# DreamOneX/yet-another-bpe

Measured on AMD Instinct MI355X. Metric: merges_per_sec, higher is better.
Workload: dtype u16

## Files before the change

include/yabpe.h:

```cpp
#ifndef YABPE_H
#define YABPE_H

#include <stddef.h>
#include <stdint.h>

#ifdef __cplusplus
extern "C" {
#endif

#define YABPE_ABI_VERSION 2

enum {
    YABPE_OK = 0,
    YABPE_E_INVALID = -1,
    YABPE_E_NODEVICE = -2,
    YABPE_E_HIP = -3,
    YABPE_E_CAPACITY = -4,
    YABPE_E_INTERNAL = -5,
    YABPE_E_COMM = -6,
    YABPE_E_UTF8 = -7
};

#define YABPE_LOAD_DEDUP 0x1u

// ... 45 lines not shown
    uint64_t retiles, table_rebuilds;
    double load_ms;
    double train_ms;
    double apply_ms_sampled;
    uint64_t apply_launches_sampled;
    uint64_t apply_algo_bytes_sampled;
    uint64_t apply_actual_bytes_sampled;
    uint64_t algo_bytes_total;
    double scan_ms_sampled;
    uint64_t scan_launches_sampled;
    uint64_t scan_algo_bytes_sampled;
    uint64_t scan_actual_bytes_sampled;
    uint64_t scan_skip_launches;
    uint64_t scan_skip_tiles_read;
    uint64_t cand_rebuilds;
    uint64_t cand_rescans;
    uint64_t fused_launches;
    double dense_ms_sampled;
    uint64_t dense_launches_sampled;
    uint64_t dense_algo_bytes_sampled;
    uint64_t dense_actual_bytes_sampled;
    double sparse_ms;
    uint64_t sparse_merges;
    double tail_ms;
    uint64_t tail_merges;
    uint64_t exchanges, exchange_bytes, exchange_cap_records, exchange_growths, exchange_max_records;
    uint64_t sparse_launches;
    uint64_t tail_launches;
    double exchange_ms_sampled;
    uint64_t exchanges_sampled;
    uint64_t exchange_p2p;
    uint64_t dense_launches, dense_merges;
    uint64_t scan_skip_pieces_taken;
} yabpe_stats_t;
int yabpe_stats(yabpe_ctx *ctx, yabpe_stats_t *out);
int yabpe_iter_log(yabpe_ctx *ctx, uint64_t *out_sites, uint64_t *out_live_slots, uint32_t cap, uint32_t *out_n);

int yabpe_event_log(yabpe_ctx *ctx, uint32_t *out_iter, float *out_us, float *out_scan_us, uint32_t cap, uint32_t *out_n);

typedef struct yabpe_latency_t {
    double launch_gap_us;
    double load_trip_us;
    double coherent_trip_us;
    double atomic_trip_us;
} yabpe_latency_t;
int yabpe_latency_probe(yabpe_ctx *ctx, yabpe_latency_t *out);

int yabpe_verify_table(yabpe_ctx *ctx, uint64_t *out_mismatches);
int yabpe_stream_checksum(yabpe_ctx *ctx, uint64_t *out_sum, uint64_t *out_words, uint64_t *out_tokens);

int yabpe_synth_generate(yabpe_ctx *ctx, uint64_t target_bytes, uint32_t n_types, uint64_t seed,
                         const uint8_t *alphabet, uint32_t alphabet_len, int space_prefix,
                         uint8_t **out_dev_bytes, uint64_t **out_dev_off, uint64_t *out_n_words, uint64_t *out_n_bytes);
int yabpe_synth_generate_lex(yabpe_ctx *ctx, uint64_t target_bytes, uint32_t n_types, uint64_t seed,
                             const uint8_t *lex_bytes, const uint64_t *lex_off,
                             uint8_t **out_dev_bytes, uint64_t **out_dev_off, uint64_t *out_n_pieces, uint64_t *out_n_bytes);
int yabpe_synth_free(yabpe_ctx *ctx);
int yabpe_memcpy_d2h(yabpe_ctx *ctx, void *dst_host, const void *src_dev, uint64_t n);
int yabpe_memcpy_h2d(yabpe_ctx *ctx, void *dst_dev, const void *src_host, uint64_t n);

int yabpe_pretokenize(yabpe_ctx *ctx, const uint8_t *text, uint64_t n_bytes, const uint64_t *chunk_off, uint32_t n_chunks,
                      const uint8_t *special_bytes, const uint32_t *special_off, uint32_t n_special,
                      const uint8_t **out_dev_text, uint64_t **out_dev_word_off, uint64_t *out_n_words, int64_t *out_bad_pos);
int yabpe_pretokenize_free(yabpe_ctx *ctx);

int yabpe_pool_add(yabpe_ctx *ctx, const uint8_t *bytes, const uint64_t *word_off, const uint64_t *word_freq, uint64_t n_words);
// ... 109 lines not shown
```

yet-another-bpe_amd/csrc/yabpe.hip:

```cpp
#include <hip/hip_runtime.h>
#include <dlfcn.h>
#include <rccl/rccl.h>

#include <algorithm>
#include <cstdarg>
#include <cstddef>
#include <cstdio>
#include <cstring>
#include <map>
#include <mutex>
#include <string>
#include <vector>

#include "../../include/yabpe.h"
#include "yabpe_kernels.h"
#include "yabpe_aux_kernels.h"
#include "yabpe_devmem.h"
#include "yabpe_pretok_kernels.h"
#include "yabpe_encode_kernels.h"
#include "yabpe_dropout_kernels.h"
#include "yabpe_decode_kernels.h"
#include "yabpe_layout_kernels.h"
#include "yabpe_replay_kernels.h"
#include "yabpe_pool_kernels.h"
// ... 61 lines not shown
}

struct yabpe_ctx {
    int device = 0;
    int n_cu = 256;
    int apply_occ = 4;
    hipStream_t stream = nullptr;
    std::string err;
    std::map<std::string, int64_t> opt;

    bool have_vocab = false;
    uint32_t base_tokens = 0;
    TokTable tt{};
    bool have_words = false;
    bool weighted = false;
    uint64_t n_words = 0, n_words_input = 0, tokens_initial = 0;
    uint32_t n_tiles = 0;
    uint16_t *tiles = nullptr, *tiles_alt = nullptr;
    uint32_t tiles_cap = 0, tiles_alt_cap = 0;
    uint32_t *tile_len = nullptr, *tile_len_alt = nullptr;
    uint32_t *tile_wbase = nullptr, *tile_wbase_alt = nullptr;
    uint32_t *wfreq = nullptr;
    uint32_t n_long = 0;
    uint16_t *long_tok = nullptr;
    unsigned long long *long_sig = nullptr;
    uint32_t long_sig_stride = 0;
    unsigned long long *long_off = nullptr;
    uint32_t *long_len = nullptr, *long_freq = nullptr;
    uint64_t long_tokens = 0;
    PairTable table{};
    uint64_t table_cap = 0;
    DevState *st = nullptr;
    DevState *st_host = nullptr;
    Best *partials = nullptr;
    uint32_t n_partials = 0, n_partials_cap = 0;
    uint32_t rec_cap = 0, rec_n = 0;
    uint32_t *rec_left = nullptr, *rec_right = nullptr, *rec_merged = nullptr;
    unsigned long long *rec_count = nullptr, *rec_sites = nullptr, *rec_live = nullptr;
    std::vector<uint64_t> log_sites, log_live;
    std::vector<uint32_t> ev_iter;
    std::vector<float> ev_us;
    yabpe_stats_t stats{};
    std::vector<EventPair> events;
    std::vector<void *> synth_bufs;
    std::vector<void *> pretok_bufs;
    uint8_t *pt_cls = nullptr;
    bool have_enc_model = false;
    unsigned long long *enc_keys = nullptr;
    uint32_t *enc_vals = nullptr;
    unsigned long long enc_mask = 0;
    uint32_t *enc_out_id = nullptr;
    uint8_t *enc_sp_bytes = nullptr, *enc_sp_has = nullptr;
    uint32_t *enc_sp_off = nullptr, *enc_sp_id = nullptr;
    uint32_t enc_n_special = 0, enc_sp_max_len = 0;
    uint32_t *enc_ids = nullptr;
    unsigned long long *enc_doc = nullptr;
    unsigned long long *enc_spans = nullptr;
    yabpe_encode_stats_t enc_stats{};
    unsigned long long enc_sums[4] = {0, 0, 0, 0};
    bool enc_done = false;
    hipEvent_t enc_ev[8] = {};
    bool have_dec_model = false;
    uint2 *dec_ent = nullptr;
    uint8_t *dec_pool = nullptr;
    uint32_t dec_n = 0;
    uint8_t *dec_text = nullptr;
    unsigned long long *dec_doc = nullptr;
    yabpe_decode_stats_t dec_stats{};
    hipEvent_t dec_ev[7] = {};
    uint32_t *lay_buf[3] = {};
    yabpe_layout_stats_t lay_stats{};
    hipEvent_t lay_ev[4] = {};
    yabpe_resume_stats_t resume_stats{};
    bool have_pool = false;
    PoolView wpool{};
    uint64_t wpool_arena_cap = 0, wpool_n = 0, wpool_bytes = 0;
    yabpe_pool_stats_t wpool_stats{};
    hipEvent_t wpool_ev[4] = {};
    unsigned long long *scratch64 = nullptr;
    unsigned long long *blk_stats = nullptr;
    uint32_t blk_used = 0;
    bool split_mode = false;
    uint32_t kmax_now = 1;
    uint32_t rec_n_live = 0;
    std::vector<float> ev_scan_us;
    unsigned long long *sig = nullptr;
    uint32_t sig_stride = 0;
    unsigned long long *blk_read = nullptr;
    uint64_t scan_skip_launches = 0;
    uint64_t piece_tag = 0;
    bool sig_valid = false;
    uint32_t sig_built_at = 0;
    uint64_t sig_tokens_at_build = 0;
    uint64_t sig_builds = 0;
    CandState *cand_state = nullptr;
    uint32_t cand_built_at = 0;
    unsigned long long cand_best_at_build = 0;
    uint32_t *sel_ticket = nullptr;
    unsigned long long *cand = nullptr;
    bool use_cand = false;
    uint64_t cand_rebuilds = 0, cand_rescans = 0;
    double cand_margin = 0.2;
    uint32_t cand_n_at_build = 0;
    bool pending = false;
    uint64_t fused_launches = 0;
    int rank = 0, n_ranks = 1;
    bool multi = false;
    ncclComm_t comm = nullptr;
    yabpe_allgather_fn ag_fn = nullptr;
    void *ag_user = nullptr;
    unsigned long long *xsmall = nullptr;
    uint8_t *xsend = nullptr, *xrecv = nullptr;
    uint64_t exchange_growths = 0;
    uint64_t exchange_max_records = 0;
    uint32_t xcap = 0;
    uint64_t xstride = 0;
    uint32_t xeff = 0;
    uint64_t xeff_sum = 0;
    uint32_t xseen[4] = {0, 0, 0, 0};
    uint64_t exchanges = 0;
    bool p2p = false;
    uint8_t *p2p_area = nullptr;
    std::vector<uint8_t *> p2p_peer;
    uint64_t p2p_half = 0, p2p_flags_off = 0, p2p_seq = 0, p2p_stride = 0;
    uint32_t p2p_cap = 0;
    hipEvent_t p2p_e0 = nullptr, p2p_e1 = nullptr;
    bool p2p_pending = false;
};
// ... 96 lines not shown
    t.sink_rec = nullptr;
    t.sink_hdr = nullptr;
    t.sink_cap = 0;
}

int table_alloc(yabpe_ctx *c, PairTable &t, uint64_t cap, unsigned long long *entries_ctr) {
    TRY(dmalloc(c, &t.keys, cap));
    TRY(dmalloc(c, &t.cnt, cap));
    t.cap = (uint32_t)cap;
    t.max_probe = c->multi ? (uint32_t)cap : (uint32_t)std::min<uint64_t>(cap, 2048);
    t.sink_rec = nullptr;
    t.sink_hdr = nullptr;
    t.sink_cap = 0;
    t.entries = entries_ctr;
    t.cand_cs = nullptr;
    t.cand_list = nullptr;
    t.cand_T = 0;
    HIPCHK(c, hipMemsetAsync(t.keys, 0xFF, cap * sizeof(uint32_t), c->stream));
    HIPCHK(c, hipMemsetAsync(t.cnt, 0, cap * sizeof(unsigned long long), c->stream));
    return 0;
}

int cand_attach(yabpe_ctx *c) {
    c->use_cand = false;
    PairTable &t = c->table;
    t.cand_cs = nullptr;
    t.cand_list = nullptr;
    if (!optv(c, "cand_argmax", 1)) return 0;
    if (!c->sel_ticket) {
        TRY(dmalloc(c, &c->sel_ticket, TICKET_WORDS));
        HIPCHK(c, hipMemsetAsync(c->sel_ticket, 0, TICKET_WORDS * 4, c->stream));
    }
    if (!c->cand_state) {
        TRY(dmalloc(c, &c->cand_state, 1));
        TRY(dmalloc(c, &c->cand, CAND_CAP));
    }
    return 0;
}

int cand_rebuild(yabpe_ctx *c, unsigned long long best_count) {
    c->use_cand = false;
    c->table.cand_cs = nullptr;
    c->table.cand_list = nullptr;
    if (!optv(c, "cand_argmax", 1) || !c->cand_state || best_count < (unsigned long long)optv(c, "cand_min_count", 16)) return 0;
    const uint32_t target = (uint32_t)std::max<int64_t>(64, optv(c, "cand_target", 768));
    const uint32_t grid = (uint32_t)std::min<uint64_t>(1024, std::max<uint64_t>(1, c->table_cap / (BLOCK * 8)));
    CandState h{};
    for (int attempt = 0; attempt < 12; ++attempt) {
        unsigned long long margin = (unsigned long long)((double)best_count * c->cand_margin);
        if (margin < 1) margin = 1;
        h = CandState{best_count - std::min(margin, best_count - 1), 0u, 0u, 0u, 0u};
        HIPCHK(c, hipMemcpyAsync(c->cand_state, &h, sizeof h, hipMemcpyHostToDevice, c->stream));
        PairTable t = c->table;
        t.cand_list = c->cand;
        t.cand_cs = c->cand_state;
        t.cand_T = h.T;
        {
            CandParams P{t, c->tt.rec, c->partials, c->st, c->cand_state, nullptr, SelectParams{}};
            hipLaunchKernelGGL(k_cand_rebuild, dim3(grid), dim3(BLOCK), 0, c->stream, P);
        }
        HIPCHK(c, hipGetLastError());
        HIPCHK(c, hipMemcpyAsync(&h, c->cand_state, sizeof h, hipMemcpyDeviceToHost, c->stream));
        HIPCHK(c, hipStreamSynchronize(c->stream));
        c->cand_rebuilds++;
        if ((h.overflow || h.n > target) && margin > 1) {
            c->cand_margin *= 0.5;
            continue;
        }
        break;
    }
    if (h.n < target / 8) c->cand_margin = std::min((double)optv(c, "cand_margin_max_pct", 60) / 100.0, c->cand_margin * 2.0);
    c->use_cand = !h.overflow && h.n < CAND_CAP / 2;
    c->cand_n_at_build = h.n;
    if (c->use_cand) {
        c->table.cand_cs = c->cand_state;
        c->table.cand_list = c->cand;
        c->table.cand_T = h.T;
    }
    return 0;
}

uint32_t count_grid(yabpe_ctx *c) {
    uint32_t want = (c->n_tiles + WPB - 1) / WPB;
    uint32_t cap = (uint32_t)optv(c, "apply_blocks", (int64_t)c->n_cu * c->apply_occ);
    return std::max(1u, std::min(std::min(want, cap), MAX_APPLY_BLOCKS));
}

int fold_stats(yabpe_ctx *c) {
    FoldParams F{c->st, c->blk_stats, std::max(c->blk_used, 1u)};
    hipLaunchKernelGGL(k_fold_stats, dim3(1), dim3(BLOCK), 0, c->stream, F);
    HIPCHK(c, hipGetLastError());
    c->blk_used = 0;
    return 0;
}

int comm_allgather(yabpe_ctx *c, const void *send, void *recv, uint64_t nbytes) {
    if (c->comm) {
        NCCLCHK(c, rccl()->AllGather(send, recv, nbytes, ncclUint8, c->comm, c->stream));
        return 0;
    }
    if (!c->ag_fn) return fail(c, YABPE_E_COMM, "no transport attached");
    HIPCHK(c, hipStreamSynchronize(c->stream));
    int rc = c->ag_fn(c->ag_user, send, recv, nbytes);
    if (rc != 0) return fail(c, YABPE_E_COMM, "custom all-gather transport failed (%d)", rc);
    return 0;
}

int comm_max(yabpe_ctx *c, unsigned long long v, unsigned long long *out);

int exchange_table(yabpe_ctx *c, PairTable lt, uint64_t lcap, PairTable t) {
    unsigned long long *d_cnt = &c->scratch64[8];
    HIPCHK(c, hipMemsetAsync(d_cnt, 0, 8, c->stream));
// ... 479 lines not shown
    return YABPE_OK;
}

void yabpe_destroy(yabpe_ctx *c) {
    if (!c) return;
    (void)hipSetDevice(c->device);
    if (c->stream) (void)hipStreamSynchronize(c->stream);
    yabpe_synth_free(c);
    yabpe_pretokenize_free(c);
    yabpe_encode_free(c);
    dfree(c->enc_keys); dfree(c->enc_vals); dfree(c->enc_out_id);
    dfree(c->enc_sp_bytes); dfree(c->enc_sp_has); dfree(c->enc_sp_off); dfree(c->enc_sp_id);
    for (auto &e : c->enc_ev)
        if (e) (void)hipEventDestroy(e);
    yabpe_decode_free(c);
    dfree(c->dec_ent); dfree(c->dec_pool);
    for (auto &e : c->dec_ev)
        if (e) (void)hipEventDestroy(e);
    yabpe_layout_free(c);
    for (auto &e : c->lay_ev)
        if (e) (void)hipEventDestroy(e);
    yabpe_pool_clear(c);
    for (auto &e : c->wpool_ev)
        if (e) (void)hipEventDestroy(e);
    dfree(c->pt_cls);
    free_corpus(c);
    free_records(c);
    dfree(c->tt.pool); dfree(c->tt.off); dfree(c->tt.len); dfree(c->tt.rec); dfree(c->tt.vset);
    dfree(c->partials);
    dfree(c->st);
    dfree(c->scratch64);
    dfree(c->blk_stats);
    dfree(c->blk_read);
    dfree(c->cand_state);
    dfree(c->sel_ticket);
    dfree(c->cand);
    dfree(c->xsend);
    dfree(c->xrecv);
    dfree(c->xsmall);
    p2p_close(c);
    if (c->p2p_e0) (void)hipEventDestroy(c->p2p_e0);
    if (c->p2p_e1) (void)hipEventDestroy(c->p2p_e1);
    if (c->comm && rccl()) (void)rccl()->CommDestroy(c->comm);
    if (c->st_host) (void)hipHostFree(c->st_host);
    for (auto &e : c->events) {
        (void)hipEventDestroy(e.e0);
        (void)hipEventDestroy(e.e1);
        (void)hipEventDestroy(e.e2);
    }
    if (c->stream) (void)hipStreamDestroy(c->stream);
    delete c;
}

int yabpe_set_option(yabpe_ctx *c, const char *name, int64_t value) {
    if (!c || !name) return YABPE_E_INVALID;
    c->opt[name] = value;
    return YABPE_OK;
}

int yabpe_set_vocab(yabpe_ctx *c, const uint8_t *tok_bytes, const uint32_t *tok_off, uint32_t n_tokens) {
    if (!c) return YABPE_E_INVALID;
    HIPCHK(c, hipSetDevice(c->device));
    if (!tok_bytes || !tok_off || n_tokens < 256) return fail(c, YABPE_E_INVALID, "vocab needs the 256 byte tokens first");
    for (uint32_t b = 0; b < 256; ++b)
        if (tok_off[b + 1] - tok_off[b] != 1 || tok_bytes[tok_off[b]] != b)
            return fail(c, YABPE_E_INVALID, "token %u must be the single byte %u (trainer.py:123-125)", b, b);
    if (n_tokens >= YB_MAX_TOKENS) return fail(c, YABPE_E_CAPACITY, "base vocabulary too large for u16 token ids");
    const uint32_t pool_cap = (uint32_t)optv(c, "pool_bytes", 64 << 20) & ~3u;
    const uint32_t vset_cap = 1u << 18;
    std::vector<uint32_t> off(n_tokens), len(n_tokens), order(n_tokens);
    std::vector<uint8_t> pool;
    for (uint32_t i = 0; i < n_tokens; ++i) {
        len[i] = tok_off[i + 1] - tok_off[i];
        off[i] = (uint32_t)pool.size();
        pool.insert(pool.end(), tok_bytes + tok_off[i], tok_bytes + tok_off[i + 1]);
        pool.resize((pool.size() + 3) & ~(size_t)3, 0);
        order[i] = i;
// ... 595 lines not shown
        if (c->rec_cap && c->rec_n_live) {
            const size_t n = c->rec_n_live;
            HIPCHK(c, hipMemcpyAsync(nl, c->rec_left, n * 4, hipMemcpyDeviceToDevice, c->stream));
            HIPCHK(c, hipMemcpyAsync(nr, c->rec_right, n * 4, hipMemcpyDeviceToDevice, c->stream));
            HIPCHK(c, hipMemcpyAsync(nm, c->rec_merged, n * 4, hipMemcpyDeviceToDevice, c->stream));
            HIPCHK(c, hipMemcpyAsync(nc, c->rec_count, n * 8, hipMemcpyDeviceToDevice, c->stream));
            HIPCHK(c, hipMemcpyAsync(ns, c->rec_sites, n * 8, hipMemcpyDeviceToDevice, c->stream));
            HIPCHK(c, hipMemcpyAsync(nv, c->rec_live, n * 8, hipMemcpyDeviceToDevice, c->stream));
        }
        HIPCHK(c, hipStreamSynchronize(c->stream));
        free_records(c);
        c->rec_left = nl; c->rec_right = nr; c->rec_merged = nm; c->rec_count = nc; c->rec_sites = ns; c->rec_live = nv;
        c->rec_cap = ncap;
        return 0;
    };
    c->rec_n_live = 0;
    const uint32_t rec_first = (uint32_t)std::min<uint64_t>(num_merges, (uint64_t)YB_MAX_TOKENS + 4096);
    if (c->rec_cap < rec_first) { free_records(c); }
    TRY(ensure_records(rec_first));
    HIPCHK(c, hipMemsetAsync(c->rec_sites, 0, (size_t)c->rec_cap * 8, c->stream));

    const uint32_t check = (uint32_t)std::max<int64_t>(1, optv(c, "check_interval", 32));
    const uint32_t ev_sample = (uint32_t)std::max<int64_t>(0, optv(c, "event_sample", 0));
    const uint32_t ev_sample_dense = (uint32_t)std::max<int64_t>(0, optv(c, "event_sample_dense", (int64_t)ev_sample));
    const double retile_frac = (double)optv(c, "retile_pct", 60) / 100.0;
    const uint64_t retile_min_tiles = (uint64_t)optv(c, "retile_min_tiles", 4096);
    size_t ev_next = 0;

    TrainEvents T;
    if (T.create() != 0) return fail(c, YABPE_E_HIP, "event creation failed");
    HIPCHK(c, hipEventRecord(T.t0, c->stream));
    bool split_marked = false, tail_marked = false;
    uint32_t split_at = 0, tail_at = 0;

    uint32_t i = 0;
    const bool trace_host = optv(c, "trace_host", 0) != 0;
#define YB_TRACE(...) do { if (trace_host) { fprintf(stderr, "[yabpe r%d] ", c->rank); fprintf(stderr, __VA_ARGS__); fprintf(stderr, "\n"); fflush(stderr); } } while (0)
    bool finished = false;
    bool skip_cand_once = false;
    bool first_round = true;
    unsigned long long prev_best = 0;
    uint64_t launches_sparse = 0, launches_at_tail = 0, launches_dense = 0, launch_no = 0;
    uint32_t dense_applied = 0;
    uint32_t cand_n_all = 0;
    bool sparse_global = false;
    c->use_cand = false;
    c->pending = false;
    while (!finished) {
        uint32_t want_partials = (uint32_t)std::min<uint64_t>(1024, std::max<uint64_t>(1, c->table_cap / (BLOCK * 8)));
        if (want_partials != c->n_partials) {
            HIPCHK(c, hipStreamSynchronize(c->stream));
            dfree(c->partials);
            c->partials = nullptr;
            c->n_partials_cap = std::max<uint32_t>(want_partials, 64);
            TRY(dmalloc(c, &c->partials, c->n_partials_cap));
            c->n_partials = want_partials;
        }
        const uint32_t apply_grid = count_grid(c);
        const int64_t split_opt = optv(c, "split", -1);
        const bool sparse_now = split_opt >= 0 ? split_opt == 1 : sparse_global;
        c->split_mode = sparse_now && c->n_tiles;
        if (!tail_marked && i >= num_merges / 2) {
            tail_marked = true;
            tail_at = i;
            launches_at_tail = launches_sparse;
            HIPCHK(c, hipEventRecord(T.t_tail, c->stream));
        }
        if (c->split_mode && !split_marked) {
            split_marked = true;
            split_at = i;
            dense_applied = i - std::min<uint32_t>(i, c->pending ? h->n_batch : 0u);
            launches_dense = h->n_select - std::min<uint32_t>(h->n_select, c->pending ? 1u : 0u);
            HIPCHK(c, hipEventRecord(T.t_split, c->stream));
        }
        if (skip_cand_once) {
            c->use_cand = false;
            skip_cand_once = false;
        } else if (h->iter > rec_base) {
            const uint32_t every = (uint32_t)std::max<int64_t>(1, optv(c, "cand_rebuild_every", 512));
            const unsigned long long drop = prev_best > h->best_count ? prev_best - h->best_count : 0;
            const bool near_T = h->best_count < c->table.cand_T + 2 * drop + 1;
            const bool long_list = cand_n_all > std::max<uint32_t>(4u * BLOCK - 64u, (uint32_t)optv(c, "cand_target", 768));
            if (!c->use_cand || i - c->cand_built_at >= every || i < c->cand_built_at || near_T || long_list) {
                YB_TRACE("cand_rebuild at %u", i);
                TRY(cand_rebuild(c, h->best_count));
                c->cand_built_at = i;
                c->cand_best_at_build = h->best_count;
            }
            prev_best = h->best_count;
        }
        if (c->split_mode) {
            const uint32_t every = (uint32_t)std::max<int64_t>(1, optv(c, "sig_rebuild_every", 16384));
            const uint64_t merged_since = c->sig_tokens_at_build > h->tokens_now ? c->sig_tokens_at_build - h->tokens_now : 0;
            const bool stale = merged_since * 100 > c->sig_tokens_at_build * (uint64_t)optv(c, "sig_rebuild_pct", 20);
            if (!c->sig_valid || i - c->sig_built_at >= every || i < c->sig_built_at || stale) {
                YB_TRACE("build_signatures at %u", i);
                TRY(build_signatures(c));
                c->sig_valid = true;
                c->sig_built_at = i;
            }
        }
        const uint32_t kmax = sparse_now ? (uint32_t)std::max<int64_t>(1, std::min<int64_t>(KMAX, optv(c, "batch_max", KMAX))) : 1u;
        if (kmax != c->kmax_now) {
            HIPCHK(c, hipMemcpyAsync(&c->st->kmax, &kmax, sizeof(uint32_t), hipMemcpyHostToDevice, c->stream));
            c->kmax_now = kmax;
            h->kmax = kmax;
        }
        const uint32_t n_launch = (first_round && !sparse_now) ? std::min<uint32_t>(check, 8) : check;
        first_round = false;
        c->rec_n_live = i;
        TRY(ensure_records((uint32_t)std::min<uint64_t>(num_merges, (uint64_t)i + (uint64_t)(n_launch + 2) * kmax)));
        auto sample = [&](uint32_t iter_rel) -> EventPair * {
            const uint32_t every = c->split_mode ? ev_sample : ev_sample_dense;
            if (!every || (launch_no++ % every) != 0) return nullptr;
            if (ev_next == c->events.size()) {
                EventPair n{};
                if (hipEventCreate(&n.e0) != hipSuccess || hipEventCreate(&n.e1) != hipSuccess || hipEventCreate(&n.e2) != hipSuccess) return nullptr;
                c->events.push_back(n);
            }
            c->events[ev_next].iter_rel = iter_rel;
            return &c->events[ev_next++];
        };
        const bool fuse = can_fuse(c);
        const uint32_t tok_upper0 = h->n_tokens;
        uint32_t launched = 0;
        if (c->pending && !fuse) {
            TRY(launch_apply(c, rec_base, tok_upper0 + kmax, apply_grid, sample(i ? i - 1 : 0), false));
            c->pending = false;
        }
        if (fuse && !c->pending && i < num_merges) {
            TRY(launch_select(c, rec_base));
            c->pending = true;
            ++i;
        }
        for (uint32_t l = 0; l < n_launch && i < num_merges + (fuse ? 1u : 0u); ++l) {
            ++launched;
            const uint32_t tok_upper = tok_upper0 + (launched + 1u) * kmax + 1u;
            if (fuse) {
                const bool last = i >= num_merges;
                TRY(launch_apply(c, rec_base, tok_upper, apply_grid, sample(i - 1), true));
                if (kmax == 1) ++i; else if (sparse_now) ++launches_sparse;
                if (last) break;
            } else {
                TRY(launch_select(c, rec_base));
                TRY(launch_apply(c, rec_base, tok_upper, apply_grid, sample(i), false));
                ++i;
            }
        }
        YB_TRACE("round of %u launches queued (p2p seq %llu), waiting", launched, (unsigned long long)c->p2p_seq);
        TRY(fold_stats(c));
        TRY(state_pull(c));
        i = h->iter - rec_base;
        YB_TRACE("round done: %u merges, halt %u req %u done %u", i, h->halt, h->halt_req, h->done);
        if (c->p2p_pending) {
            float xms = 0;
            if (hipEventElapsedTime(&xms, c->p2p_e0, c->p2p_e1) == hipSuccess) {
                c->stats.exchange_ms_sampled += xms;
                c->stats.exchanges_sampled += 1;
            } else {
                (void)hipGetLastError();
            }
            c->p2p_pending = false;
        }
        if (h->halt_req && !h->halt) h->halt = h->halt_req;
        if (h->done || h->halt) c->pending = false;
        if (c->multi && c->xrecv) {
            const uint32_t seen = h->xmax;
            c->exchange_max_records = std::max<uint64_t>(c->exchange_max_records, seen);
            c->xseen[3] = c->xseen[2]; c->xseen[2] = c->xseen[1]; c->xseen[1] = c->xseen[0]; c->xseen[0] = seen;
            if (optv(c, "delta_adapt", 1) && h->halt != HALT_DELTA_FULL && h->iter - rec_base >= 4 * check) {
                const uint64_t recent = std::max(std::max(c->xseen[0], c->xseen[1]), std::max(c->xseen[2], c->xseen[3]));
                const uint64_t gran = (uint64_t)std::max<int64_t>(1, optv(c, "delta_granule", 1024));
                const uint64_t raw = recent * (uint64_t)std::max<int64_t>(1, optv(c, "delta_headroom_pct", 200)) / 100ull + (uint64_t)std::max<int64_t>(0, optv(c, "delta_margin", 1024));
                const uint64_t want = ((raw + gran - 1) / gran) * gran;
                c->xeff = (uint32_t)std::min<uint64_t>(c->xcap, std::max<uint64_t>(want, std::min<uint64_t>((uint64_t)std::max<int64_t>(1, optv(c, "delta_floor", 2048)), c->xcap)));
            }
            if (optv(c, "trace_exchange", 0) && c->rank == 0) fprintf(stderr, "[yabpe] exchange: merges %u records<= %u next %u halt %u\n", h->iter - rec_base, seen, c->xeff, h->halt);
            HIPCHK(c, hipMemsetAsync(&c->st->xmax, 0, sizeof(uint32_t), c->stream));
            h->xmax = 0;
        }
        cand_n_all = h->cand_n;
        unsigned long long want_sparse = (c->n_tiles && h->iter > rec_base &&
                 (c->weighted && h->sites ? h->sites : h->best_count) * 100 < (unsigned long long)c->n_tiles * (unsigned long long)optv(c, "split_pct", 100)) ? 1 : 0;
        if (c->multi) {
// ... 49 lines not shown
                return fail(c, YABPE_E_COMM, "a peer's records did not arrive within the time limit (peer-to-peer exchange) after %u merges; rank %d launched exchange %llu, "
                            "flags in its receive area [half][sender]: %s", h->iter - rec_base, c->rank, (unsigned long long)c->p2p_seq, seen.c_str());
            }
            const char *why = h->halt == HALT_POOL_FULL ? "token byte pool exhausted (option pool_bytes)"
                              : h->halt == HALT_VOCAB_FULL ? "u16 token id space exhausted"
                                                           : "device halt";
            return fail(c, YABPE_E_CAPACITY, "%s after %u merges", why, h->iter - rec_base);
        }
        if (h->done || (i >= num_merges && !c->pending)) {
            finished = true;
            break;
        }
        if (h->table_entries * 100 > c->table_cap * (uint64_t)optv(c, "table_load_pct", 30))
        {
            YB_TRACE("table_grow");
            TRY(table_grow(c, std::max<uint64_t>(h->table_entries * (uint64_t)std::max<int64_t>(2, optv(c, "table_grow_x", 8)), 1ull << 16)));
            YB_TRACE("table_grow back");
        }
        if (c->n_tiles >= retile_min_tiles && !c->weighted &&
            (double)h->live_slots < retile_frac * (double)c->n_tiles * SPAN) {
            YB_TRACE("retile");
            TRY(retile_flat(c));
        }
    }
    HIPCHK(c, hipEventRecord(T.t1, c->stream));
    HIPCHK(c, hipEventSynchronize(T.t1));
    float ms = 0;
    HIPCHK(c, hipEventElapsedTime(&ms, T.t0, T.t1));
    if (split_marked) {
        float sms = 0;
        HIPCHK(c, hipEventElapsedTime(&sms, T.t_split, T.t1));
        c->stats.sparse_ms += sms;
        c->stats.sparse_merges += (h->iter - rec_base) > split_at ? (h->iter - rec_base) - split_at : 0;
        c->stats.sparse_launches += launches_sparse;
    }
    if (tail_marked) {
        float tms = 0;
        HIPCHK(c, hipEventElapsedTime(&tms, T.t_tail, T.t1));
        c->stats.tail_ms += tms;
        c->stats.tail_merges += (h->iter - rec_base) > tail_at ? (h->iter - rec_base) - tail_at : 0;
        c->stats.tail_launches += launches_sparse - launches_at_tail;
    }
    c->stats.train_ms += ms;

    TRY(state_pull(c));
    const uint32_t n = h->iter - rec_base;
    c->rec_n = n;
    c->log_sites.assign(n, 0);
    c->log_live.assign(n, 0);
    if (n) {
        HIPCHK(c, hipMemcpy(c->log_sites.data(), c->rec_sites, (size_t)n * 8, hipMemcpyDeviceToHost));
        HIPCHK(c, hipMemcpy(c->log_live.data(), c->rec_live, (size_t)n * 8, hipMemcpyDeviceToHost));
        c->log_sites[n - 1] += h->sites;
    }
    const uint64_t tokens_at_start = h->tokens_now - h->sites + [&] { uint64_t s = 0; for (uint32_t k = 0; k < n; ++k) s += c->log_sites[k]; return s; }();
    h->tokens_now -= h->sites;
    h->sites = 0;
    TRY(state_push(c));
    {
        uint64_t T_ = tokens_at_start;
        std::vector<uint64_t> Ti(n);
        for (uint32_t k = 0; k < n; ++k) {
            Ti[k] = T_;
            c->stats.algo_bytes_total += 2 * (T_ + c->n_words_input);
            T_ -= c->log_sites[k];
        }
        if (!split_marked) {
            dense_applied = n - std::min<uint32_t>(n, (c->pending && !h->done) ? h->n_batch : 0u);
            launches_dense = h->n_select - std::min<uint32_t>(h->n_select, (c->pending && !h->done) ? 1u : 0u);
        }
        dense_applied = std::min(dense_applied, n);
        uint64_t dense_algo = 0, dense_actual = 0, dense_sampled_now = 0;
        for (uint32_t k = 0; k < dense_applied; ++k) {
            dense_algo += 2 * (Ti[k] + c->n_words_input);
// ... 1425 lines not shown
```

yet-another-bpe_amd/csrc/yabpe_kernels.h:

```cpp
#pragma once
#include <hip/hip_runtime.h>
#include <stdint.h>

#include <type_traits>

#include "limit_logic.h"
#include "steal_logic.h"
#include "tile_logic.h"

namespace yb {

constexpr int CAP = 1024;
constexpr int LMAX = 64;
constexpr int SPAN = CAP - LMAX + 1;
constexpr int WPB = 4;
constexpr int BLOCK = WPB * 64;
constexpr int AGG_N = 1024;
constexpr uint32_t EMPTY = 0xFFFFFFFFu;
constexpr uint32_t PADPAD = (YB_PAD << 16) | YB_PAD;
constexpr int LONG_CH = 1024;
constexpr int SIG_ROWS = 512;
constexpr int SIG_ROWS_LOG2 = 9;
constexpr int SIG_TILES = 8;
constexpr int MAX_LISTS_PROF = 4096;
// ... 1613 lines not shown
    __shared__ unsigned long long s_fold[2];
    if (threadIdx.x < 2) s_fold[threadIdx.x] = 0;
    __syncthreads();
    unsigned long long a = 0, f = 0;
    for (uint32_t i = threadIdx.x; i < n_blk; i += BLOCK) {
        a += blk[2 * i];
        f += blk[2 * i + 1];
        blk[2 * i] = 0;
        blk[2 * i + 1] = 0;
    }
    for (int o = 32; o >= 1; o >>= 1) {
        a += __shfl_xor(a, o);
        f += __shfl_xor(f, o);
    }
    if ((threadIdx.x & 63) == 0 && (a | f)) {
        atomicAdd(&s_fold[0], a);
        atomicAdd(&s_fold[1], f);
    }
    __syncthreads();
    if (threadIdx.x == 0) {
        st->sites += s_fold[0];
        st->live_slots -= s_fold[1];
    }
    __syncthreads();
}

struct FoldParams {
    DevState *st;
    unsigned long long *blk_stats;
    uint32_t n_blk;
};
__global__ __launch_bounds__(BLOCK) void k_fold_stats(FoldParams P) { fold_block_stats(P.st, P.blk_stats, P.n_blk); }


#ifdef YB_PROFILE_SCAN
__device__ unsigned long long g_stop_hist[65536];
#define YB_STOP(it, why, n, nw) do { if (lane == 0) g_stop_hist[(it) & 0xFFFFu] = (unsigned long long)(why) | ((unsigned long long)(n) << 8) | ((unsigned long long)(nw) << 16); } while (0)
__device__ unsigned long long g_launch_prof[65536 * 4];
__device__ unsigned long long g_sel_prof[16];
__device__ unsigned long long g_sel_acc[3 * 24];
#define YB_SEL_STAMP(i) do { if (threadIdx.x == 0) g_sel_prof[i] = wall_clock64(); } while (0)
#else
#define YB_SEL_STAMP(i) do { } while (0)
#define YB_STOP(it, why, n, nw) do { } while (0)
#endif
template <int NF = 4>
__device__ __forceinline__ Best cand_list_best(const PairTable &t, const TokRec *rec, uint32_t n, uint32_t first, uint32_t step) {
    Best best{0ull, 0u, EMPTY, 0u, 0u};
    for (uint32_t i0 = first; i0 < n; i0 += (uint32_t)NF * step) {
        unsigned long long e[NF], cn[NF];
        uint32_t rl[NF], rr[NF];
#pragma unroll
        for (int k = 0; k < NF; ++k) {
            const uint32_t i = i0 + (uint32_t)k * step;
            e[k] = i < n ? ld_coherent(&t.cand_list[i]) : ~0ull;
        }
#pragma unroll
        for (int k = 0; k < NF; ++k) {
            cn[k] = 0ull;
            if (i0 + (uint32_t)k * step < n) {
                const uint32_t key = (uint32_t)(e[k] >> 32);
                cn[k] = ld_coherent(pt_count_ptr(t, e[k]));
                rl[k] = ld_coherent(&rec[key >> 16].rank);
                rr[k] = ld_coherent(&rec[key & 0xffffu].rank);
            }
        }
// ... 763 lines not shown
        Best best = cand_list_best(P.table, P.rec, min(P.cs->n, CAND_CAP), blockIdx.x * BLOCK + threadIdx.x, gridDim.x * BLOCK);
        best = best_wave_reduce(best);
        const int lane = threadIdx.x & 63, wib = threadIdx.x >> 6;
        if (lane == 0) s_b[wib] = best;
        __syncthreads();
        if (threadIdx.x == 0) {
            for (int i = 1; i < WPB; ++i)
                if (best_gt(s_b[i], best)) best = s_b[i];
            best_store_coherent(&P.partials[blockIdx.x], best);
        }
#ifdef YB_PROFILE_SCAN
        if (blockIdx.x == 0) YB_SEL_STAMP(9);
#endif
    }
    if (!last_workgroup(P.ticket)) return;
    select_body(P.sel);
}

__global__ __launch_bounds__(BLOCK) void k_cand_rebuild(CandParams P) {
    const unsigned long long T = P.cs->T;
    for (uint32_t s = blockIdx.x * BLOCK + threadIdx.x; s < P.table.cap; s += gridDim.x * BLOCK) {
        const long long cn = (long long)P.table.cnt[s];
        if (cn <= 0 || (unsigned long long)cn < T) continue;
        const uint32_t idx = atomicAdd(&P.cs->n, 1u);
        if (idx < CAND_CAP) P.table.cand_list[idx] = (unsigned long long)s | ((unsigned long long)P.table.keys[s] << 32); else P.cs->overflow = 1u;
    }
}

struct BatchLds {
    uint32_t a[KMAX], b[KMAX], c[KMAX];
    uint32_t row[KMAX];
    unsigned long long mask[KMAX];
};

template <bool WEIGHTED, bool HIST = false>
__global__ __launch_bounds__(BLOCK) void k_apply(ApplyParams P, uint32_t apply_blocks, RankParams R, FuseParams F, LongParams LW, uint32_t long_first) {
    using AggV = typename std::conditional<WEIGHTED, unsigned long long, int>::type;
    static_assert(!(HIST && WEIGHTED), "the direct-indexed store holds 32-bit deltas");
    __shared__ uint32_t s_keys[HIST ? 1 : AGG_N];
    __shared__ AggV s_vals[HIST ? 1 : AGG_N];
    __shared__ int s_hist[HIST ? 4 * HIST_V : 1];
    __shared__ __attribute__((aligned(16))) WaveLds s_w[WPB];
    __shared__ unsigned long long s_cnt[2];

    DevState *st = P.st;
    if (st->done | st->halt) return;
    if (blockIdx.x >= long_first) {
        apply_long_block(LW, blockIdx.x - long_first);
    } else if (blockIdx.x >= apply_blocks) {
        rank_update_block(R, blockIdx.x - apply_blocks);
    } else {
    const int lane = threadIdx.x & 63;
    const int wib = __builtin_amdgcn_readfirstlane(threadIdx.x >> 6);
    SlowCtx<AggV> C{P, Agg<AggV>{s_keys, s_vals, HIST ? 0u : (uint32_t)AGG_N - 1u}, st, st->a, st->b, st->c, 0u, 0u, lane,
                    KeyMemo{{EMPTY, EMPTY, EMPTY, EMPTY}, {0u, 0u, 0u, 0u}}, HIST ? s_hist : nullptr};
    C.mk = yb_memkey(C.a, C.b);
    C.self = yb_pairkey(C.a, C.b);
    const uint32_t mk = C.mk;
    if constexpr (HIST) hist_init(Hist{s_hist}); else agg_init(C.agg);
    if (threadIdx.x < 2) s_cnt[threadIdx.x] = 0;
    WaveLds &W = s_w[wib];
    wave_lds_init(W, lane);
    __syncthreads();

    unsigned long long wave_sites = 0;
    unsigned long long wave_freed = 0;
// ... 567 lines not shown
```

yet-another-bpe_amd/yet_another_bpe/_native.py:

```python
from __future__ import annotations

import ctypes
import os
from ctypes import POINTER, byref, c_char_p, c_double, c_int, c_int64, c_uint8, c_uint32, c_uint64, c_void_p
from pathlib import Path

import numpy as np

_CSRC = Path(__file__).resolve().parent.parent / "csrc"
LIB_PATH = Path(os.environ.get("YABPE_LIB", _CSRC / "libyabpe.so"))


class YabpeError(RuntimeError):
    def __init__(self, code: int, msg: str):
        super().__init__(f"yabpe error {code}: {msg}")
        self.code = code


class Utf8Error(ValueError):

    def __init__(self, position: int):
        super().__init__(f"invalid UTF-8 at byte {position}")
        self.position = position


E_CAPACITY = -4
E_UTF8 = -7


class Stats(ctypes.Structure):
    _fields_ = [(n, c_uint64) for n in (
        "n_words", "n_words_input", "n_long_words", "tokens_initial", "tokens_now", "merges_done", "n_tiles",
        "live_slots", "table_capacity", "table_entries", "retiles", "table_rebuilds")] + [
        ("load_ms", c_double), ("train_ms", c_double), ("apply_ms_sampled", c_double)] + [(n, c_uint64) for n in (
            "apply_launches_sampled", "apply_algo_bytes_sampled", "apply_actual_bytes_sampled", "algo_bytes_total")] + [
        ("scan_ms_sampled", c_double)] + [(n, c_uint64) for n in (
            "scan_launches_sampled", "scan_algo_bytes_sampled", "scan_actual_bytes_sampled", "scan_skip_launches", "scan_skip_tiles_read", "cand_rebuilds", "cand_rescans", "fused_launches")] + [
        ("dense_ms_sampled", c_double)] + [(n, c_uint64) for n in ("dense_launches_sampled", "dense_algo_bytes_sampled", "dense_actual_bytes_sampled")] + [
        ("sparse_ms", c_double), ("sparse_merges", c_uint64), ("tail_ms", c_double), ("tail_merges", c_uint64)] + [
        (n, c_uint64) for n in ("exchanges", "exchange_bytes", "exchange_cap_records", "exchange_growths", "exchange_max_records", "sparse_launches", "tail_launches")] + [("exchange_ms_sampled", c_double), ("exchanges_sampled", c_uint64), ("exchange_p2p", c_uint64),
        ("dense_launches", c_uint64), ("dense_merges", c_uint64), ("scan_skip_pieces_taken", c_uint64)]


class EncodeStats(ctypes.Structure):
    _fields_ = [(n, c_uint64) for n in ("n_bytes", "n_docs", "n_pretokens", "n_unique", "n_unique_long", "n_specials", "n_ids")] + [
        (n, c_double) for n in ("split_ms", "pretok_ms", "pool_ms", "words_ms", "emit_ms", "total_ms")]


class DecodeStats(ctypes.Structure):
    _fields_ = [(n, c_uint64) for n in ("n_ids", "n_docs", "n_unknown", "n_gathered", "n_bytes", "n_replacements", "n_docs_repaired")] + [
        (n, c_double) for n in ("lengths_ms", "gather_ms", "check_ms", "repair_ms", "total_ms")]


class LayoutStats(ctypes.Structure):
    _fields_ = [(n, c_uint64) for n in ("n_ids", "n_docs", "n_rows", "row_len", "n_truncated_docs", "n_ids_dropped", "n_pad_slots")] + [
        (n, c_double) for n in ("lengths_ms", "write_ms", "total_ms")]


class Layout(ctypes.Structure):
    _fields_ = [(n, c_uint32) for n in ("row_len", "pad_id", "bos_id", "eos_id", "flags")]


class ResumeStats(ctypes.Structure):
    _fields_ = [(n, c_uint64) for n in ("n_unique", "n_long", "tokens")] + [(n, c_double) for n in ("segment_ms", "build_ms")]


class PoolStats(ctypes.Structure):
    _fields_ = [(n, c_uint64) for n in ("n_calls", "n_words_added", "n_empty_dropped", "n_unique", "n_bytes", "slot_capacity",
                                        "arena_capacity", "slot_growths", "arena_growths")] + [
        (n, c_double) for n in ("pool_ms", "probe_ms", "append_ms", "total_ms")]


class Latency(ctypes.Structure):
    _fields_ = [(n, c_double) for n in ("launch_gap_us", "load_trip_us", "coherent_trip_us", "atomic_trip_us")]
# ... 585 lines not shown
```

Before: 48390.

## Pipeline sparse training rounds with mapped-memory snapshots and queued candidate rebuilds

Adds a double-buffered round pipeline for the fused sparse phase. A snapshot kernel folds block stats and copies device state plus candidate state into pinned host memory, and an event marks each snapshot, so the host can queue the next round before reading the previous one instead of synchronizing every round. Candidate-list rebuilds become a single queued kernel writing into alternating slots, with margin retries decided from a later snapshot. The cost is one round of lag: records, token bounds and near-threshold checks are widened to cover it, drains happen on halt, table load or retile, and the control logic is more complex.

```diff
diff --git a/include/yabpe.h b/include/yabpe.h
--- a/include/yabpe.h
+++ b/include/yabpe.h
@@ -101,6 +101,7 @@
     uint64_t exchange_p2p;
     uint64_t dense_launches, dense_merges;
     uint64_t scan_skip_pieces_taken;
+    uint64_t rounds_pipelined, round_drains;
 } yabpe_stats_t;
 int yabpe_stats(yabpe_ctx *ctx, yabpe_stats_t *out);
 int yabpe_iter_log(yabpe_ctx *ctx, uint64_t *out_sites, uint64_t *out_live_slots, uint32_t cap, uint32_t *out_n);
diff --git a/yet-another-bpe_amd/csrc/yabpe.hip b/yet-another-bpe_amd/csrc/yabpe.hip
--- a/yet-another-bpe_amd/csrc/yabpe.hip
+++ b/yet-another-bpe_amd/csrc/yabpe.hip
@@ -117,6 +117,8 @@
     uint64_t table_cap = 0;
     DevState *st = nullptr;
     DevState *st_host = nullptr;
+    RoundSnap *snap_host = nullptr;
+    hipEvent_t snap_ev[2] = {nullptr, nullptr};
     Best *partials = nullptr;
     uint32_t n_partials = 0, n_partials_cap = 0;
     uint32_t rec_cap = 0, rec_n = 0;
@@ -179,6 +181,8 @@
     uint64_t sig_tokens_at_build = 0;
     uint64_t sig_builds = 0;
     CandState *cand_state = nullptr;
+    CandState *cand_slots = nullptr;
+    bool cand_idle_clean = false;
     uint32_t cand_built_at = 0;
     unsigned long long cand_best_at_build = 0;
     uint32_t *sel_ticket = nullptr;
@@ -341,7 +345,9 @@
         HIPCHK(c, hipMemsetAsync(c->sel_ticket, 0, TICKET_WORDS * 4, c->stream));
     }
     if (!c->cand_state) {
-        TRY(dmalloc(c, &c->cand_state, 1));
+        TRY(dmalloc(c, &c->cand_slots, 2));
+        c->cand_state = c->cand_slots;
+        c->cand_idle_clean = false;
         TRY(dmalloc(c, &c->cand, CAND_CAP));
     }
     return 0;
@@ -387,6 +393,37 @@
         c->table.cand_T = h.T;
     }
     return 0;
+}
+
+int cand_rebuild_queued(yabpe_ctx *c, unsigned long long best_count, bool *margin_gt1) {
+    unsigned long long margin = (unsigned long long)((double)best_count * c->cand_margin);
+    if (margin < 1) margin = 1;
+    *margin_gt1 = margin > 1;
+    const unsigned long long T = best_count - std::min(margin, best_count - 1);
+    const uint32_t grid = (uint32_t)std::min<uint64_t>(1024, std::max<uint64_t>(1, c->table_cap / (BLOCK * 8)));
+    CandState *slot = c->cand_slots + (c->cand_state == c->cand_slots ? 1 : 0);
+    if (!c->cand_idle_clean) HIPCHK(c, hipMemsetAsync(slot, 0, sizeof(CandState), c->stream));
+    c->cand_state = slot;
+    c->cand_idle_clean = false;
+    c->table.cand_list = c->cand;
+    c->table.cand_cs = c->cand_state;
+    c->table.cand_T = T;
+    CandParams P{c->table, c->tt.rec, c->partials, c->st, c->cand_state, nullptr, SelectParams{}};
+    hipLaunchKernelGGL(k_cand_rebuild_slot, dim3(grid), dim3(BLOCK), 0, c->stream, P, T);
+    HIPCHK(c, hipGetLastError());
+    c->cand_rebuilds++;
+    c->use_cand = true;
+    return 0;
+}
+bool cand_rebuild_result(yabpe_ctx *c, const CandState &h, bool margin_gt1) {
+    const uint32_t target = (uint32_t)std::max<int64_t>(64, optv(c, "cand_target", 768));
+    c->cand_n_at_build = h.n;
+    if ((h.overflow || h.n > target) && margin_gt1) {
+        c->cand_margin *= 0.5;
+        return true;
+    }
+    if (h.n < target / 8) c->cand_margin = std::min((double)optv(c, "cand_margin_max_pct", 60) / 100.0, c->cand_margin * 2.0);
+    return h.overflow || h.n >= CAND_CAP / 2;
 }
 
 uint32_t count_grid(yabpe_ctx *c) {
@@ -932,7 +969,7 @@
     dfree(c->scratch64);
     dfree(c->blk_stats);
     dfree(c->blk_read);
-    dfree(c->cand_state);
+    dfree(c->cand_slots);
     dfree(c->sel_ticket);
     dfree(c->cand);
     dfree(c->xsend);
@@ -943,6 +980,9 @@
     if (c->p2p_e1) (void)hipEventDestroy(c->p2p_e1);
     if (c->comm && rccl()) (void)rccl()->CommDestroy(c->comm);
     if (c->st_host) (void)hipHostFree(c->st_host);
+    if (c->snap_host) (void)hipHostFree(c->snap_host);
+    for (auto &e : c->snap_ev)
+        if (e) (void)hipEventDestroy(e);
     for (auto &e : c->events) {
         (void)hipEventDestroy(e.e0);
         (void)hipEventDestroy(e.e1);
@@ -1604,6 +1644,7 @@
     HIPCHK(c, hipEventRecord(T.t0, c->stream));
     bool split_marked = false, tail_marked = false;
     uint32_t split_at = 0, tail_at = 0;
+    uint32_t n_select_split = 0, n_select_tail = 0;
 
     uint32_t i = 0;
     const bool trace_host = optv(c, "trace_host", 0) != 0;
@@ -1618,6 +1659,46 @@
     bool sparse_global = false;
     c->use_cand = false;
     c->pending = false;
+#ifdef YB_PROFILE_SCAN
+    bool pipe_on = false;
+#else
+    bool pipe_on = optv(c, "round_pipeline", 1) != 0 && !c->multi && ev_sample == 0;
+#endif
+    if (pipe_on && !c->snap_host) {
+        HIPCHK(c, hipHostMalloc((void **)&c->snap_host, 2 * sizeof(RoundSnap), hipHostMallocDefault));
+        memset(c->snap_host, 0, 2 * sizeof(RoundSnap));
+        for (auto &e : c->snap_ev) HIPCHK(c, hipEventCreate(&e));
+    }
+    RoundSnap *snap_dev = nullptr;
+    if (pipe_on) HIPCHK(c, hipHostGetDevicePointer((void **)&snap_dev, c->snap_host, 0));
+    uint32_t snap_seq = 0;
+    uint32_t snaps_out = 0;
+    bool pipe_started = false;
+    bool cand_queued = false, cand_queued_gt1 = false, cand_retry = false;
+    uint32_t cand_queued_seq = 0;
+    const unsigned long long cand_min_count = (unsigned long long)optv(c, "cand_min_count", 16);
+    auto pipe_ok = [&]() {
+        return pipe_on && c->split_mode && !skip_cand_once && h->iter > rec_base && c->cand_state && optv(c, "fused", 1) && optv(c, "cand_argmax", 1) &&
+               optv(c, "skip_index", 1) && h->best_count >= cand_min_count;
+    };
+    auto table_loaded = [&]() { return h->table_entries * 100 > c->table_cap * (uint64_t)optv(c, "table_load_pct", 30); };
+    auto retile_due = [&]() {
+        return c->n_tiles >= retile_min_tiles && !c->weighted && (double)h->live_slots < retile_frac * (double)c->n_tiles * SPAN;
+    };
+    auto cand_result = [&](const CandState &cs) {
+        if (cand_rebuild_result(c, cs, cand_queued_gt1)) {
+            cand_retry = true;
+            if (!cand_queued_gt1) pipe_on = false;
+        }
+        cand_queued = false;
+    };
+    auto snap_read = [&](uint32_t seq) -> int {
+        HIPCHK(c, hipEventSynchronize(c->snap_ev[seq & 1u]));
+        const RoundSnap &s = c->snap_host[seq & 1u];
+        *h = s.st;
+        if (cand_queued && (int32_t)(seq - cand_queued_seq) >= 0) cand_result(s.cs);
+        return 0;
+    };
     while (!finished) {
         uint32_t want_partials = (uint32_t)std::min<uint64_t>(1024, std::max<uint64_t>(1, c->table_cap / (BLOCK * 8)));
         if (want_partials != c->n_partials) {
@@ -1636,32 +1717,48 @@
             tail_marked = true;
             tail_at = i;
             launches_at_tail = launches_sparse;
+            n_select_tail = h->n_select;
             HIPCHK(c, hipEventRecord(T.t_tail, c->stream));
         }
         if (c->split_mode && !split_marked) {
             split_marked = true;
             split_at = i;
+            n_select_split = h->n_select;
             dense_applied = i - std::min<uint32_t>(i, c->pending ? h->n_batch : 0u);
             launches_dense = h->n_select - std::min<uint32_t>(h->n_select, c->pending ? 1u : 0u);
             HIPCHK(c, hipEventRecord(T.t_split, c->stream));
         }
-        if (skip_cand_once) {
+        const bool pipe_round = pipe_ok();
+        bool rescan_round = false;
+        if (snaps_out && !pipe_round) return fail(c, YABPE_E_INTERNAL, "a round is queued and the next one cannot follow it");
+        if (pipe_started) {
+        } else if (skip_cand_once) {
             c->use_cand = false;
             skip_cand_once = false;
+            rescan_round = true;
         } else if (h->iter > rec_base) {
             const uint32_t every = (uint32_t)std::max<int64_t>(1, optv(c, "cand_rebuild_every", 512));
             const unsigned long long drop = prev_best > h->best_count ? prev_best - h->best_count : 0;
-            const bool near_T = h->best_count < c->table.cand_T + 2 * drop + 1;
+            const bool near_T = h->best_count < c->table.cand_T + (pipe_round ? 3 : 2) * drop + 1;
             const bool long_list = cand_n_all > std::max<uint32_t>(4u * BLOCK - 64u, (uint32_t)optv(c, "cand_target", 768));
-            if (!c->use_cand || i - c->cand_built_at >= every || i < c->cand_built_at || near_T || long_list) {
-                YB_TRACE("cand_rebuild at %u", i);
-                TRY(cand_rebuild(c, h->best_count));
+            if (!c->use_cand || i - c->cand_built_at >= every || i < c->cand_built_at || near_T || long_list || cand_retry) {
+                YB_TRACE("cand_rebuild at %u%s", i, pipe_round ? " (queued)" : "");
+                cand_retry = false;
+                if (pipe_round) {
+                    const unsigned long long best_then = h->best_count - (snaps_out ? std::min(drop, h->best_count - 1) : 0ull);
+                    TRY(cand_rebuild_queued(c, best_then, &cand_queued_gt1));
+                    cand_queued = true;
+                    cand_queued_seq = snap_seq;
+                } else {
+                    cand_queued = false;
+                    TRY(cand_rebuild(c, h->best_count));
+                }
                 c->cand_built_at = i;
                 c->cand_best_at_build = h->best_count;
             }
             prev_best = h->best_count;
         }
-        if (c->split_mode) {
+        if (c->split_mode && !pipe_started) {
             const uint32_t every = (uint32_t)std::max<int64_t>(1, optv(c, "sig_rebuild_every", 16384));
             const uint64_t merged_since = c->sig_tokens_at_build > h->tokens_now ? c->sig_tokens_at_build - h->tokens_now : 0;
             const bool stale = merged_since * 100 > c->sig_tokens_at_build * (uint64_t)optv(c, "sig_rebuild_pct", 20);
@@ -1678,10 +1775,12 @@
             c->kmax_now = kmax;
             h->kmax = kmax;
         }
-        const uint32_t n_launch = (first_round && !sparse_now) ? std::min<uint32_t>(check, 8) : check;
+        const uint32_t n_launch = (first_round && !sparse_now) ? std::min<uint32_t>(check, 8) : (rescan_round && !c->multi) ? 1u : check;
         first_round = false;
-        c->rec_n_live = i;
-        TRY(ensure_records((uint32_t)std::min<uint64_t>(num_merges, (uint64_t)i + (uint64_t)(n_launch + 2) * kmax)));
+        pipe_started = false;
+        const uint32_t lag = snaps_out ? n_launch * kmax : 0u;
+        c->rec_n_live = (uint32_t)std::min<uint64_t>(c->rec_cap, (uint64_t)i + lag);
+        TRY(ensure_records((uint32_t)std::min<uint64_t>(num_merges, (uint64_t)i + lag + (uint64_t)(n_launch + 2) * kmax)));
         auto sample = [&](uint32_t iter_rel) -> EventPair * {
             const uint32_t every = c->split_mode ? ev_sample : ev_sample_dense;
             if (!every || (launch_no++ % every) != 0) return nullptr;
@@ -1694,7 +1793,9 @@
             return &c->events[ev_next++];
         };
         const bool fuse = can_fuse(c);
-        const uint32_t tok_upper0 = h->n_tokens;
+        const bool steady = pipe_round && fuse && c->split_mode;
+        if (snaps_out && !steady) return fail(c, YABPE_E_INTERNAL, "a round is queued and this one is not of the fused sparse form");
+        const uint32_t tok_upper0 = h->n_tokens + lag;
         uint32_t launched = 0;
         if (c->pending && !fuse) {
             TRY(launch_apply(c, rec_base, tok_upper0 + kmax, apply_grid, sample(i ? i - 1 : 0), false));
@@ -1720,8 +1821,39 @@
             }
         }
         YB_TRACE("round of %u launches queued (p2p seq %llu), waiting", launched, (unsigned long long)c->p2p_seq);
-        TRY(fold_stats(c));
-        TRY(state_pull(c));
+        if (steady) {
+            SnapParams SP{FoldParams{c->st, c->blk_stats, std::max(c->blk_used, 1u)}, c->cand_state,
+                          c->cand_slots + (c->cand_state == c->cand_slots ? 1 : 0), snap_dev + (snap_seq & 1u)};
+            c->cand_idle_clean = true;
+            hipLaunchKernelGGL(k_round_snapshot, dim3(1), dim3(BLOCK), 0, c->stream, SP);
+            HIPCHK(c, hipGetLastError());
+            c->blk_used = 0;
+            HIPCHK(c, hipEventRecord(c->snap_ev[snap_seq & 1u], c->stream));
+            ++snap_seq;
+            ++snaps_out;
+            if (snaps_out == 1) {
+                pipe_started = true;
+                continue;
+            }
+            TRY(snap_read(snap_seq - snaps_out));
+            --snaps_out;
+            c->stats.rounds_pipelined++;
+            const bool need_drain = h->halt || h->halt_req || (!h->done && (!pipe_ok() || table_loaded() || retile_due()));
+            if (need_drain) {
+                YB_TRACE("queue drained (halt %u req %u)", h->halt, h->halt_req);
+                TRY(snap_read(snap_seq - 1u));
+                snaps_out = 0;
+                c->stats.round_drains++;
+            }
+        } else {
+            TRY(fold_stats(c));
+            TRY(state_pull(c));
+            if (cand_queued) {
+                CandState cs{};
+                HIPCHK(c, hipMemcpy(&cs, c->cand_state, sizeof cs, hipMemcpyDeviceToHost));
+                cand_result(cs);
+            }
+        }
         i = h->iter - rec_base;
         YB_TRACE("round done: %u merges, halt %u req %u done %u", i, h->halt, h->halt_req, h->done);
         if (c->p2p_pending) {
@@ -1837,14 +1969,16 @@
         HIPCHK(c, hipEventElapsedTime(&sms, T.t_split, T.t1));
         c->stats.sparse_ms += sms;
         c->stats.sparse_merges += (h->iter - rec_base) > split_at ? (h->iter - rec_base) - split_at : 0;
-        c->stats.sparse_launches += launches_sparse;
+        const uint64_t worked = h->n_select > n_select_split ? h->n_select - n_select_split : 0;
+        c->stats.sparse_launches += snap_seq ? std::min<uint64_t>(launches_sparse, worked) : launches_sparse;
     }
     if (tail_marked) {
         float tms = 0;
         HIPCHK(c, hipEventElapsedTime(&tms, T.t_tail, T.t1));
         c->stats.tail_ms += tms;
         c->stats.tail_merges += (h->iter - rec_base) > tail_at ? (h->iter - rec_base) - tail_at : 0;
-        c->stats.tail_launches += launches_sparse - launches_at_tail;
+        const uint64_t worked = h->n_select > n_select_tail ? h->n_select - n_select_tail : 0;
+        c->stats.tail_launches += snap_seq ? std::min<uint64_t>(launches_sparse - launches_at_tail, worked) : launches_sparse - launches_at_tail;
     }
     c->stats.train_ms += ms;
 
diff --git a/yet-another-bpe_amd/csrc/yabpe_kernels.h b/yet-another-bpe_amd/csrc/yabpe_kernels.h
--- a/yet-another-bpe_amd/csrc/yabpe_kernels.h
+++ b/yet-another-bpe_amd/csrc/yabpe_kernels.h
@@ -1669,6 +1669,27 @@
 };
 __global__ __launch_bounds__(BLOCK) void k_fold_stats(FoldParams P) { fold_block_stats(P.st, P.blk_stats, P.n_blk); }
 
+struct RoundSnap {
+    DevState st;
+    CandState cs;
+};
+struct SnapParams {
+    FoldParams fold;
+    const CandState *cs;
+    CandState *cs_idle;
+    RoundSnap *out;
+};
+__global__ __launch_bounds__(BLOCK) void k_round_snapshot(SnapParams P) {
+    fold_block_stats(P.fold.st, P.fold.blk_stats, P.fold.n_blk);
+    static_assert(sizeof(DevState) % 4 == 0 && sizeof(CandState) % 4 == 0, "copied as 32-bit words");
+    const uint32_t *src = reinterpret_cast<const uint32_t *>(P.fold.st);
+    uint32_t *dst = reinterpret_cast<uint32_t *>(&P.out->st);
+    for (uint32_t i = threadIdx.x; i < sizeof(DevState) / 4; i += BLOCK) dst[i] = ld_coherent(src + i);
+    const uint32_t *csrc = reinterpret_cast<const uint32_t *>(P.cs);
+    uint32_t *cdst = reinterpret_cast<uint32_t *>(&P.out->cs);
+    for (uint32_t i = threadIdx.x; i < sizeof(CandState) / 4; i += BLOCK) cdst[i] = ld_coherent(csrc + i);
+    if (threadIdx.x == 0) *P.cs_idle = CandState{0ull, 0u, 0u, 0u, 0u};
+}
 
 #ifdef YB_PROFILE_SCAN
 __device__ unsigned long long g_stop_hist[65536];
@@ -2498,6 +2519,16 @@
     uint32_t row[KMAX];
     unsigned long long mask[KMAX];
 };
+
+__global__ __launch_bounds__(BLOCK) void k_cand_rebuild_slot(CandParams P, unsigned long long T) {
+    if (blockIdx.x == 0 && threadIdx.x == 0) P.cs->T = T;
+    for (uint32_t s = blockIdx.x * BLOCK + threadIdx.x; s < P.table.cap; s += gridDim.x * BLOCK) {
+        const long long cn = (long long)P.table.cnt[s];
+        if (cn <= 0 || (unsigned long long)cn < T) continue;
+        const uint32_t idx = atomicAdd(&P.cs->n, 1u);
+        if (idx < CAND_CAP) P.table.cand_list[idx] = (unsigned long long)s | ((unsigned long long)P.table.keys[s] << 32); else P.cs->overflow = 1u;
+    }
+}
 
 template <bool WEIGHTED, bool HIST = false>
 __global__ __launch_bounds__(BLOCK) void k_apply(ApplyParams P, uint32_t apply_blocks, RankParams R, FuseParams F, LongParams LW, uint32_t long_first) {
diff --git a/yet-another-bpe_amd/yet_another_bpe/_native.py b/yet-another-bpe_amd/yet_another_bpe/_native.py
--- a/yet-another-bpe_amd/yet_another_bpe/_native.py
+++ b/yet-another-bpe_amd/yet_another_bpe/_native.py
@@ -39,7 +39,8 @@
         ("dense_ms_sampled", c_double)] + [(n, c_uint64) for n in ("dense_launches_sampled", "dense_algo_bytes_sampled", "dense_actual_bytes_sampled")] + [
         ("sparse_ms", c_double), ("sparse_merges", c_uint64), ("tail_ms", c_double), ("tail_merges", c_uint64)] + [
         (n, c_uint64) for n in ("exchanges", "exchange_bytes", "exchange_cap_records", "exchange_growths", "exchange_max_records", "sparse_launches", "tail_launches")] + [("exchange_ms_sampled", c_double), ("exchanges_sampled", c_uint64), ("exchange_p2p", c_uint64),
-        ("dense_launches", c_uint64), ("dense_merges", c_uint64), ("scan_skip_pieces_taken", c_uint64)]
+        ("dense_launches", c_uint64), ("dense_merges", c_uint64), ("scan_skip_pieces_taken", c_uint64),
+        ("rounds_pipelined", c_uint64), ("round_drains", c_uint64)]
 
 
 class EncodeStats(ctypes.Structure):
```

Result: no change. 48440, median of 4 (+0.1%).
